# vitasoftAI/ImageRetrievalResearch

Hardware: AMD Instinct MI355X
Metric: images/sec embed + queries/sec top-k@100k-gallery, EffNet-B3a 224^2 (higher is better)
Workload: dtype bf16

## Files before the change

imageretrievalresearch_amd/csrc/common.h:

```cpp
#pragma once
#include <hip/hip_runtime.h>
#include <hip/hip_bf16.h>
#include <stdint.h>
#include <stdio.h>
#include <string>

namespace mi355 {

void set_error(const char* fmt, ...);
void roctx_enable(bool on);
bool roctx_active();
void roctx_push(const char* label);
void roctx_pop();
struct RoctxRange {
    bool on;
    explicit RoctxRange(const char* label) : on(label && roctx_active()) { if (on) roctx_push(label); }
    ~RoctxRange() { if (on) roctx_pop(); }
};
enum { OK = 0, ERR_ARG = 1, ERR_HIP = 2, ERR_STATE = 3, ERR_UNSUPPORTED = 4 };

#define MI355_CHECK_HIP(expr)                                                              \
    do {                                                                                   \
        hipError_t _e = (expr);                                                            \
        if (_e != hipSuccess) {                                                            \
            mi355::set_error("%s:%d: %s -> %s", __FILE__, __LINE__, #expr, hipGetErrorString(_e)); \
            return mi355::ERR_HIP;                                                         \
        }                                                                                  \
    } while (0)

#define MI355_REQUIRE(cond, ...)                                                           \
    do {                                                                                   \
        if (!(cond)) {                                                                     \
            mi355::set_error(__VA_ARGS__);                                                 \
            return mi355::ERR_ARG;                                                         \
        }                                                                                  \
    } while (0)

#define MI355_LAUNCH_CHECK() MI355_CHECK_HIP(hipGetLastError())

constexpr int MI355_MAX_DEVICES = 64;
static inline bool first_time_on_this_device(bool* flags) {
    int dev = 0;
    if (hipGetDevice(&dev) != hipSuccess || dev < 0 || dev >= MI355_MAX_DEVICES) return true;
    if (flags[dev]) return false;
    flags[dev] = true;
    return true;
}

static inline int cdiv(long a, long b) { return (int)((a + b - 1) / b); }
static inline size_t align_up(size_t a, size_t b) { return (a + b - 1) / b * b; }

static inline char* align256(const void* p) { return (char*)(((uintptr_t)p + 255) & ~(uintptr_t)255); }
struct WsCarver {
    char* base;
    size_t off = 0;
    explicit WsCarver(void* ws) : base(ws ? align256(ws) : nullptr) {}
    char* next() const { return base ? base + off : nullptr; }
    char* take(size_t bytes) { char* p = next(); off += align_up(bytes, 256); return p; }
    size_t total() const { return off + 256; }
};

typedef unsigned short bf16_t;

__device__ __forceinline__ float bf2f(bf16_t v) { return __uint_as_float(((unsigned)v) << 16); }
__device__ __forceinline__ bf16_t f2bf(float f) {
    __hip_bfloat16 h = __float2bfloat16(f);
    return *reinterpret_cast<bf16_t*>(&h);
}
typedef __bf16 mi355_bf16x2 __attribute__((ext_vector_type(2)));
typedef float mi355_f32x2 __attribute__((ext_vector_type(2)));
__device__ __forceinline__ unsigned pack2bf(float lo, float hi) {
    const mi355_bf16x2 v = __builtin_convertvector((mi355_f32x2){lo, hi}, mi355_bf16x2);
    return *reinterpret_cast<const unsigned*>(&v);
}

__device__ __forceinline__ float sigmoid_f(float x) {
    return __builtin_amdgcn_rcpf(1.0f + __builtin_amdgcn_exp2f(-1.4426950408889634f * x));
}
__device__ __forceinline__ float silu_f(float x) { return x * sigmoid_f(x); }

__device__ __forceinline__ float gelu_f(float x) {
    const float z = fabsf(x) * 0.70710678118654752f;
    const float t = __builtin_amdgcn_rcpf(1.0f + 0.3275911f * z);
    const float poly = ((((1.061405429f * t - 1.453152027f) * t + 1.421413741f) * t - 0.284496736f) * t + 0.254829592f) * t;
    const float e = 1.0f - poly * __builtin_amdgcn_exp2f(-1.4426950408889634f * z * z);
    return 0.5f * x * (1.0f + copysignf(e, x));
}

enum Act { ACT_NONE = 0, ACT_SILU = 1, ACT_RELU = 2, ACT_RELU6 = 3, ACT_GELU = 4, ACT_SIGMOID = 5 };

__device__ __forceinline__ float apply_act(float x, int act) {
    switch (act) {
        case ACT_SILU: return silu_f(x);
        case ACT_RELU: return fmaxf(x, 0.f);
        case ACT_RELU6: return fminf(fmaxf(x, 0.f), 6.f);
        case ACT_GELU: return gelu_f(x);
        case ACT_SIGMOID: return sigmoid_f(x);
        default: return x;
    }
}

template <int ACT>
__device__ __forceinline__ float act_c(float x) {
    if constexpr (ACT == ACT_SILU) return silu_f(x);
    else if constexpr (ACT == ACT_RELU) return fmaxf(x, 0.f);
    else if constexpr (ACT == ACT_RELU6) return fminf(fmaxf(x, 0.f), 6.f);
    else if constexpr (ACT == ACT_GELU) return gelu_f(x);
    else if constexpr (ACT == ACT_SIGMOID) return sigmoid_f(x);
    else return x;
}
#define MI355_ACT_DISPATCH(act_runtime, ...)                                      \
    switch (act_runtime) {                                                        \
        case ::mi355::ACT_SILU: { constexpr int ACT = ::mi355::ACT_SILU; __VA_ARGS__ } break;   \
        case ::mi355::ACT_GELU: { constexpr int ACT = ::mi355::ACT_GELU; __VA_ARGS__ } break;   \
        case ::mi355::ACT_RELU6: { constexpr int ACT = ::mi355::ACT_RELU6; __VA_ARGS__ } break; \
        case ::mi355::ACT_RELU: { constexpr int ACT = ::mi355::ACT_RELU; __VA_ARGS__ } break;   \
        case ::mi355::ACT_SIGMOID: { constexpr int ACT = ::mi355::ACT_SIGMOID; __VA_ARGS__ } break; \
        default: { constexpr int ACT = ::mi355::ACT_NONE; __VA_ARGS__ } break;    \
    }

__device__ __forceinline__ float wave_sum(float v) {
#pragma unroll
    for (int o = 32; o > 0; o >>= 1) v += __shfl_xor(v, o, 64);
    return v;
}
__device__ __forceinline__ float wave_max(float v) {
#pragma unroll
    for (int o = 32; o > 0; o >>= 1) v = fmaxf(v, __shfl_xor(v, o, 64));
    return v;
}

}
```

imageretrievalresearch_amd/csrc/conv_kernels.hip:

```cpp
#include "ops.h"
#include "../../include/mi355_retrieval.h"

#include <stdlib.h>
#include <type_traits>

namespace mi355 {

typedef float f32x4 __attribute__((ext_vector_type(4)));
typedef unsigned u32x4 __attribute__((ext_vector_type(4)));
typedef unsigned u32x2 __attribute__((ext_vector_type(2)));

__device__ __forceinline__ void unpack8(u32x4 v, float* f) {
    f[0] = __uint_as_float(v.x << 16); f[1] = __uint_as_float(v.x & 0xffff0000u);
    f[2] = __uint_as_float(v.y << 16); f[3] = __uint_as_float(v.y & 0xffff0000u);
    f[4] = __uint_as_float(v.z << 16); f[5] = __uint_as_float(v.z & 0xffff0000u);
    f[6] = __uint_as_float(v.w << 16); f[7] = __uint_as_float(v.w & 0xffff0000u);
}
__device__ __forceinline__ u32x4 pack8(const float* f) {
    u32x4 o;
    o.x = pack2bf(f[0], f[1]); o.y = pack2bf(f[2], f[3]); o.z = pack2bf(f[4], f[5]); o.w = pack2bf(f[6], f[7]);
    return o;
}

constexpr int STEM_TW = 16, STEM_TH = 16;
// ... 322 lines not shown
            }
        }
    }

    if (pool_partial != nullptr) {
#pragma unroll
        for (int j = 0; j < 8; ++j) red[threadIdx.x][j] = psum[j];
        __syncthreads();
        const int ncg = CG < 256 ? CG : 256;
        if ((int)threadIdx.x < ncg) {
            float s[8];
#pragma unroll
            for (int j = 0; j < 8; ++j) s[j] = 0.f;
            for (int u = threadIdx.x; u < 256; u += CG) {
#pragma unroll
                for (int j = 0; j < 8; ++j) s[j] += red[u][j];
            }
            const int my_cg = (int)(((long)blk * 256 + threadIdx.x) % CG);
            float* pp = pool_partial + ((size_t)b * nblk + blk) * C + my_cg * 8;
            *reinterpret_cast<f32x4*>(pp) = (f32x4){s[0], s[1], s[2], s[3]};
            *reinterpret_cast<f32x4*>(pp + 4) = (f32x4){s[4], s[5], s[6], s[7]};
        }
        if (CG > 256) {
            const int first = (int)(((long)blk * 256) % CG);
            for (int t = 256 + threadIdx.x; t < CG; t += 256) {
                const int z = (first + t) % CG;
                float* pp = pool_partial + ((size_t)b * nblk + blk) * C + z * 8;
                *reinterpret_cast<f32x4*>(pp) = (f32x4){0.f, 0.f, 0.f, 0.f};
                *reinterpret_cast<f32x4*>(pp + 4) = (f32x4){0.f, 0.f, 0.f, 0.f};
            }
        }
    }
}

template <int KS, int PX>
__global__ __launch_bounds__(256) void k_dw_tiled(const bf16_t* __restrict__ in, const bf16_t* __restrict__ w,
                                                  const float* __restrict__ bias, bf16_t* __restrict__ out,
                                                  float* __restrict__ pool_partial, int H, int W, int C, int TH, int CGC,
                                                  int nbands, int act) {
    constexpr int PAD = KS / 2;
    constexpr int IW = PX - 1 + KS;
    extern __shared__ __attribute__((aligned(16))) bf16_t tile[];
    const int b = blockIdx.y;
    const int band = blockIdx.x % nbands, chunk = blockIdx.x / nbands;
    const int oy0 = band * TH;
    const int th = min(TH, H - oy0);
    const int IH = TH + KS - 1, EW = W + 2 * PAD + (PX - 1);
    const int cg0 = chunk * CGC;
    const int CG = C >> 3;
    const int ncg = min(CGC, CG - cg0);
    const int PS = CGC * 8;
    const bf16_t* inb = in + (size_t)b * H * W * C;
    for (int id = threadIdx.x; id < IH * EW * CGC; id += 256) {
        const int cg = id % CGC;
        const int px = id / CGC;
        const int r = px / EW, x = px - r * EW;
        const int iy = oy0 - PAD + r, ix = x - PAD;
        u32x4 v = {0u, 0u, 0u, 0u};
        if (cg < ncg && iy >= 0 && iy < H && ix >= 0 && ix < W)
            v = *reinterpret_cast<const u32x4*>(inb + ((size_t)iy * W + ix) * C + (cg0 + cg) * 8);
        *reinterpret_cast<u32x4*>(&tile[(size_t)px * PS + cg * 8]) = v;
    }
    __syncthreads();

    const int strips = (W + PX - 1) / PX;
    const int nitems = CGC * strips * th;
    float psum[8];
#pragma unroll
    for (int j = 0; j < 8; ++j) psum[j] = 0.f;
    for (int item = threadIdx.x; item < nitems; item += 256) {
        const int cg = item % CGC;
        const int rest = item / CGC;
        const int sx = rest % strips, oyl = rest / strips;
        if (cg >= ncg) continue;
        const int ox0 = sx * PX;
        const int c0 = (cg0 + cg) * 8;
        float acc[PX][8];
        {
            const f32x4 b0 = *reinterpret_cast<const f32x4*>(bias + c0);
            const f32x4 b1 = *reinterpret_cast<const f32x4*>(bias + c0 + 4);
#pragma unroll
            for (int p = 0; p < PX; ++p) {
                acc[p][0] = b0.x; acc[p][1] = b0.y; acc[p][2] = b0.z; acc[p][3] = b0.w;
                acc[p][4] = b1.x; acc[p][5] = b1.y; acc[p][6] = b1.z; acc[p][7] = b1.w;
            }
        }
#pragma unroll
        for (int ky = 0; ky < KS; ++ky) {
            float wk[KS][8];
#pragma unroll
            for (int kx = 0; kx < KS; ++kx)
                unpack8(*reinterpret_cast<const u32x4*>(w + (size_t)(ky * KS + kx) * C + c0), wk[kx]);
            const bf16_t* row = tile + ((size_t)(oyl + ky) * EW + ox0) * PS + cg * 8;
#pragma unroll
            for (int i = 0; i < IW; ++i) {
                float v[8];
                unpack8(*reinterpret_cast<const u32x4*>(row + (size_t)i * PS), v);
#pragma unroll
                for (int p = 0; p < PX; ++p) {
                    const int kx = i - p;
                    if (kx >= 0 && kx < KS) {
#pragma unroll
                        for (int j = 0; j < 8; ++j) acc[p][j] += wk[kx][j] * v[j];
                    }
                }
            }
        }
        MI355_ACT_DISPATCH(act, {
_Pragma("unroll")
            for (int p = 0; p < PX; ++p)
_Pragma("unroll")
                for (int j = 0; j < 8; ++j) acc[p][j] = act_c<ACT>(acc[p][j]);
        })
        bf16_t* o = out + (((size_t)b * H + oy0 + oyl) * W + ox0) * C + c0;
#pragma unroll
        for (int p = 0; p < PX; ++p) {
            if (ox0 + p < W) {
#pragma unroll
                for (int j = 0; j < 8; ++j) psum[j] += acc[p][j];
                *reinterpret_cast<u32x4*>(o + (size_t)p * C) = pack8(acc[p]);
            }
        }
    }
    if (pool_partial != nullptr) {
        __syncthreads();
        float* red = reinterpret_cast<float*>(tile);
#pragma unroll
        for (int j = 0; j < 8; ++j) red[threadIdx.x * 8 + j] = psum[j];
        __syncthreads();
        if ((int)threadIdx.x < ncg) {
            float sacc[8] = {0.f, 0.f, 0.f, 0.f, 0.f, 0.f, 0.f, 0.f};
            for (int u = threadIdx.x; u < 256; u += CGC) {
#pragma unroll
                for (int j = 0; j < 8; ++j) sacc[j] += red[u * 8 + j];
            }
            float* pp = pool_partial + ((size_t)b * nbands + band) * C + (cg0 + threadIdx.x) * 8;
            *reinterpret_cast<f32x4*>(pp) = (f32x4){sacc[0], sacc[1], sacc[2], sacc[3]};
            *reinterpret_cast<f32x4*>(pp + 4) = (f32x4){sacc[4], sacc[5], sacc[6], sacc[7]};
        }
    }
}

static bool dw_tiled_plan(int H, int W, int C, int k, int stride, int* TH, int* CGC, int* PX, size_t* lds) {
    if (stride != 1 || W < 14 || C % 8) return false;
    const int CG = C / 8;
    const int cgc = CG < 8 ? CG : 8;
    const int px = W % 7 == 0 ? 7 : 4;
    const int strips = (W + px - 1) / px;
    int th = 256 / (cgc * strips);
    if (th < 1) return false;
    if (th > H) th = H;
    const int pad = k / 2;
    const size_t bytes = (size_t)(th + k - 1) * (W + 2 * pad + px - 1) * cgc * 16;
    if (bytes > 64 * 1024 || bytes < 256 * 8 * 4) return false;
    *TH = th; *CGC = cgc; *PX = px; *lds = bytes;
    return true;
}

template <int KS, int PX>
static int launch_dw_tiled(const bf16_t* in, const bf16_t* w, const float* bias, bf16_t* out, float* pool_partial, int B,
                           int H, int W, int C, int TH, int CGC, size_t lds, int act, int* pool_nblk, hipStream_t st) {
    static bool attr_done[MI355_MAX_DEVICES] = {false};
    if (first_time_on_this_device(attr_done)) {
        MI355_CHECK_HIP(hipFuncSetAttribute((const void*)k_dw_tiled<KS, PX>, hipFuncAttributeMaxDynamicSharedMemorySize,
                                            64 * 1024));
    }
    const int nbands = cdiv(H, TH), nchunks = cdiv(C / 8, CGC);
    hipLaunchKernelGGL((k_dw_tiled<KS, PX>), dim3(nbands * nchunks, B), dim3(256), lds, st, in, w, bias, out, pool_partial,
                       H, W, C, TH, CGC, nbands, act);
    MI355_LAUNCH_CHECK();
    if (pool_nblk) *pool_nblk = nbands;
    return OK;
}

typedef __bf16 dw_bf16x8 __attribute__((ext_vector_type(8)));
template <int NU>
__global__ __launch_bounds__(256, NU >= 6 ? 2 : (NU >= 4 ? 3 : 4)) void k_dw3_lds(
    const bf16_t* __restrict__ in, const bf16_t* __restrict__ w, const float* __restrict__ bias, bf16_t* __restrict__ out,
    float* __restrict__ pool_partial, int B, int nblk, int H, int W, int act, unsigned magicW, int tiles_per_wg) {
    constexpr int C = NU * 8, PB = C * 2;
    constexpr int ROWB = 34 * PB;
    constexpr int NCH = 3 * ROWB / 16;
    constexpr int NLD = (NCH + 63) / 64;
    constexpr int OUTB = 32 * PB, NOC = OUTB / 16, NST = (NOC + 63) / 64;
    constexpr int WS = 3 * ROWB + OUTB + NU * 16 + NU * 32;
    __shared__ __attribute__((aligned(16))) unsigned char lds[4 * WS];
    __shared__ float red[4][NU * 8];
    const int xcd = blockIdx.x & 7, seq = blockIdx.x >> 3;
    const int b = xcd + 8 * (seq / nblk), blk = seq - (seq / nblk) * nblk;
    if (b >= B) return;
    const int lane = threadIdx.x & 63;
    const int wave = __builtin_amdgcn_readfirstlane(threadIdx.x >> 6);
    const int fr = lane & 15, fq = lane >> 4;
    const int HW = H * W;
    unsigned char* Lw = lds + wave * WS;
    unsigned char* Lo = Lw + 3 * ROWB;
    unsigned char* Lz = Lo + OUTB;
    float* Lb = reinterpret_cast<float*>(Lz + NU * 16);
    if (lane < NU) *reinterpret_cast<u32x4*>(Lz + lane * 16) = (u32x4){0u, 0u, 0u, 0u};
    if (lane < NU * 8) Lb[lane] = bias[lane];
    u32x4 dwf[NU][3];
    {
        const int pm = fr >> 3, c = fr & 7, t = fq - pm;
        const int q = c >> 1;
#pragma unroll
        for (int u = 0; u < NU; ++u)
#pragma unroll
            for (int ky = 0; ky < 3; ++ky) {
                unsigned v = 0u;
                if (t >= 0 && t < 3) v = w[(size_t)(ky * 3 + t) * C + u * 8 + c];
                const unsigned word = (c & 1) ? (v << 16) : v;
                dwf[u][ky] = (u32x4){q == 0 ? word : 0u, q == 1 ? word : 0u, q == 2 ? word : 0u, q == 3 ? word : 0u};
            }
    }
    const int ch4 = (fq & 1) * 4, pp = fq >> 1;
    const bf16_t* img = in + (size_t)b * HW * C;
    const __amdgpu_buffer_rsrc_t rsrc = __builtin_amdgcn_make_buffer_rsrc(const_cast<bf16_t*>(img), 0, HW * PB, 0x00020000);
    unsigned char* ob = reinterpret_cast<unsigned char*>(out + (size_t)b * HW * C);
    const int rowb = W * PB;
    const int ntiles = (HW + 31) >> 5;
    const int t_end = min(ntiles, (blk + 1) * tiles_per_wg);
    float psum[NU][4];
#pragma unroll
    for (int u = 0; u < NU; ++u)
#pragma unroll
        for (int j = 0; j < 4; ++j) psum[u][j] = 0.f;
    int s_goff[NLD], s_loff[NLD];
#pragma unroll
    for (int i = 0; i < NLD; ++i) {
        const int ch = lane + 64 * i;
        const int ky = ch / (ROWB / 16), rem = ch - ky * (ROWB / 16);
        s_loff[i] = ch < NCH ? ky * ROWB + rem * 16 : -1;
        s_goff[i] = ch < NCH ? (ky - 1) * rowb + rem * 16 - PB : 0x40000000;
    }
    u32x4 sv[NLD];
    auto stage_load = [&](int tile) {
        const int base = tile * 32 * PB;
#pragma unroll
        for (int i = 0; i < NLD; ++i) sv[i] = __builtin_amdgcn_raw_buffer_load_b128(rsrc, base + s_goff[i], 0, 0);
        __builtin_amdgcn_sched_barrier(0);
    };
    const int t_begin = blk * tiles_per_wg + wave;
    if (t_begin < t_end) stage_load(t_begin);
    for (int tile = t_begin; tile < t_end; tile += 4) {
#pragma unroll
        for (int i = 0; i < NLD; ++i)
            if (s_loff[i] >= 0) *reinterpret_cast<u32x4*>(Lw + s_loff[i]) = sv[i];
        if (tile + 4 < t_end) stage_load(tile + 4);
        const int q = tile * 32 + 2 * fr;
        const int y = (int)__umulhi((unsigned)q, magicW);
        const int x = q - y * W;
        const bool colok = !(fq == 0 && x == 0) && !(fq == 3 && x == W - 2);
        const unsigned char* rb = Lw + (2 * fr + fq) * PB;
        const unsigned char* r0 = colok ? rb : Lz;
        const unsigned char* r1 = colok ? rb + ROWB : Lz;
        const unsigned char* r2 = colok ? rb + 2 * ROWB : Lz;
        const bool live = q + pp < HW;
#pragma unroll
        for (int u = 0; u < NU; ++u) {
            const u32x4 x0 = *reinterpret_cast<const u32x4*>(r0 + u * 16);
            const u32x4 x1 = *reinterpret_cast<const u32x4*>(r1 + u * 16);
            const u32x4 x2 = *reinterpret_cast<const u32x4*>(r2 + u * 16);
            f32x4 acc = *reinterpret_cast<const f32x4*>(Lb + u * 8 + ch4);
            acc = __builtin_amdgcn_mfma_f32_16x16x32_bf16(*reinterpret_cast<const dw_bf16x8*>(&dwf[u][0]), *reinterpret_cast<const dw_bf16x8*>(&x0), acc, 0, 0, 0);
            acc = __builtin_amdgcn_mfma_f32_16x16x32_bf16(*reinterpret_cast<const dw_bf16x8*>(&dwf[u][1]), *reinterpret_cast<const dw_bf16x8*>(&x1), acc, 0, 0, 0);
            acc = __builtin_amdgcn_mfma_f32_16x16x32_bf16(*reinterpret_cast<const dw_bf16x8*>(&dwf[u][2]), *reinterpret_cast<const dw_bf16x8*>(&x2), acc, 0, 0, 0);
            MI355_ACT_DISPATCH(act, {
                acc.x = act_c<ACT>(acc.x); acc.y = act_c<ACT>(acc.y); acc.z = act_c<ACT>(acc.z); acc.w = act_c<ACT>(acc.w);
            })
            if (live) { psum[u][0] += acc.x; psum[u][1] += acc.y; psum[u][2] += acc.z; psum[u][3] += acc.w; }
            u32x2 o;
            o.x = pack2bf(acc.x, acc.y);
            o.y = pack2bf(acc.z, acc.w);
            *reinterpret_cast<u32x2*>(Lo + (2 * fr + pp) * PB + u * 16 + ch4 * 2) = o;
        }
        const int nvalid = min(32, HW - tile * 32) * PB;
#pragma unroll
        for (int i = 0; i < NST; ++i) {
            const int ob_off = (lane + 64 * i) * 16;
            if (ob_off < nvalid && ob_off < OUTB)
                *reinterpret_cast<u32x4*>(ob + (size_t)tile * 32 * PB + ob_off) = *reinterpret_cast<const u32x4*>(Lo + ob_off);
        }
    }
    if (pool_partial) {
#pragma unroll
        for (int u = 0; u < NU; ++u) {
#pragma unroll
            for (int o = 1; o < 16; o <<= 1) {
#pragma unroll
                for (int j = 0; j < 4; ++j) psum[u][j] += __shfl_xor(psum[u][j], o, 64);
            }
#pragma unroll
            for (int j = 0; j < 4; ++j) psum[u][j] += __shfl_xor(psum[u][j], 32, 64);
            if (fr == 0 && fq < 2)
                *reinterpret_cast<f32x4*>(&red[wave][u * 8 + ch4]) = (f32x4){psum[u][0], psum[u][1], psum[u][2], psum[u][3]};
        }
        __syncthreads();
        if (threadIdx.x < NU * 8)
            pool_partial[((size_t)b * nblk + blk) * C + threadIdx.x] =
                ((red[0][threadIdx.x] + red[1][threadIdx.x]) + red[2][threadIdx.x]) + red[3][threadIdx.x];
    }
}

template <int NU>
static void launch_dw3_lds(const bf16_t* in, const bf16_t* w, const float* bias, bf16_t* out, float* pool_partial, int B, int nb,
                           int H, int W, int act, unsigned magic, int tpw, hipStream_t st) {
    hipLaunchKernelGGL((k_dw3_lds<NU>), dim3((unsigned)(8 * cdiv(B, 8) * nb)), dim3(256), 0, st, in, w, bias, out, pool_partial, B,
                       nb, H, W, act, magic, tpw);
}

bool dw_tiled_supported(int H, int W, int C, int k, int stride) {
    int TH, CGC, PX;
    size_t lds;
    return dw_tiled_plan(H, W, C, k, stride, &TH, &CGC, &PX, &lds);
}

bool dw3_lds_supported(int H, int W, int C, int k, int stride) {
    return k == 3 && stride == 1 && C <= 48 && W % 2 == 0 && W >= 4 && (long)H * W * C * 2 < (1L << 30);
}

void dw_env_choice(bool* try_tiled, bool* try_mfma) {
    static const int use_tiled = getenv("MI355_DW_TILED") ? atoi(getenv("MI355_DW_TILED")) : 0;
    static const int use_mfma = getenv("MI355_DW_MFMA") ? atoi(getenv("MI355_DW_MFMA")) : 1;
    *try_tiled = use_tiled != 0;
    *try_mfma = use_mfma != 0;
}

int launch_dwconv_sel(const bf16_t* in, const bf16_t* w, const float* bias, bf16_t* out, float* pool_partial, int B, int H,
                      int W, int C, int k, int stride, int act, bool try_tiled, bool try_mfma, int* pool_nblk, int* path,
                      hipStream_t st) {
    MI355_REQUIRE(C % 8 == 0, "dwconv: C=%d must be a multiple of 8", C);
    MI355_REQUIRE((k == 3 || k == 5) && (stride == 1 || stride == 2), "dwconv: unsupported k=%d stride=%d", k, stride);
    const int pad = k / 2;
    const int Ho = (H + 2 * pad - k) / stride + 1, Wo = (W + 2 * pad - k) / stride + 1;
    auto ran = [path](int p, int e) {
        if (path && e == OK) *path = p;
        return e;
    };
    int TH, CGC, PX;
    size_t lds;
    if (try_tiled && dw_tiled_plan(H, W, C, k, stride, &TH, &CGC, &PX, &lds)) {
        const int p = MI355_DW_PATH(MI355_DW_PATH_TILED, k, 1, PX, 0);
        if (k == 3) return ran(p, PX == 7 ? launch_dw_tiled<3, 7>(in, w, bias, out, pool_partial, B, H, W, C, TH, CGC, lds, act, pool_nblk, st)
                                          : launch_dw_tiled<3, 4>(in, w, bias, out, pool_partial, B, H, W, C, TH, CGC, lds, act, pool_nblk, st));
        return ran(p, PX == 7 ? launch_dw_tiled<5, 7>(in, w, bias, out, pool_partial, B, H, W, C, TH, CGC, lds, act, pool_nblk, st)
                              : launch_dw_tiled<5, 4>(in, w, bias, out, pool_partial, B, H, W, C, TH, CGC, lds, act, pool_nblk, st));
    }
    if (try_mfma && dw3_lds_supported(H, W, C, k, stride)) {
        const int ntiles = cdiv((long)H * W, 32);
        int nb = std::min(std::min(dw_pool_blocks(Ho, Wo, C), 14), ntiles);
        const int tpw = cdiv(ntiles, nb);
        nb = cdiv(ntiles, tpw);
        if (pool_nblk) *pool_nblk = nb;
        const unsigned magic = (unsigned)((0x100000000ULL + (unsigned)W - 1) / (unsigned)W);
        switch (C / 8) {
            case 1: launch_dw3_lds<1>(in, w, bias, out, pool_partial, B, nb, H, W, act, magic, tpw, st); break;
            case 2: launch_dw3_lds<2>(in, w, bias, out, pool_partial, B, nb, H, W, act, magic, tpw, st); break;
            case 3: launch_dw3_lds<3>(in, w, bias, out, pool_partial, B, nb, H, W, act, magic, tpw, st); break;
            case 4: launch_dw3_lds<4>(in, w, bias, out, pool_partial, B, nb, H, W, act, magic, tpw, st); break;
            case 5: launch_dw3_lds<5>(in, w, bias, out, pool_partial, B, nb, H, W, act, magic, tpw, st); break;
            default: launch_dw3_lds<6>(in, w, bias, out, pool_partial, B, nb, H, W, act, magic, tpw, st); break;
        }
        MI355_LAUNCH_CHECK();
        return ran(MI355_DW_PATH(MI355_DW_PATH_LDS3, 3, 1, C / 8, 0), OK);
    }
    if (pool_nblk) *pool_nblk = dw_pool_blocks(Ho, Wo, C);
    const int nblk = dw_pool_blocks(Ho, Wo, C);
    dim3 grid((unsigned)(8 * cdiv(B, 8) * nblk));
#define DW_LAUNCH(KS, S)                                                                                            \
    hipLaunchKernelGGL((k_dwconv<KS, S>), grid, dim3(256), 0, st, in, w, bias, out, pool_partial, B, nblk, H, W, C, Ho, Wo, act)
    if (k == 3 && stride == 1) DW_LAUNCH(3, 1);
    else if (k == 3 && stride == 2) DW_LAUNCH(3, 2);
    else if (k == 5 && stride == 1) DW_LAUNCH(5, 1);
    else DW_LAUNCH(5, 2);
#undef DW_LAUNCH
    MI355_LAUNCH_CHECK();
    return ran(MI355_DW_PATH(MI355_DW_PATH_DIRECT, k, stride, DW_PX, 0), OK);
}

int launch_dwconv(const bf16_t* in, const bf16_t* w, const float* bias, bf16_t* out, float* pool_partial, int B, int H,
                  int W, int C, int k, int stride, int act, int* pool_nblk, hipStream_t st) {
    bool try_tiled, try_mfma;
    dw_env_choice(&try_tiled, &try_mfma);
    return launch_dwconv_sel(in, w, bias, out, pool_partial, B, H, W, C, k, stride, act, try_tiled, try_mfma, pool_nblk, nullptr, st);
}

constexpr int SE_THREADS = 1024;
__global__ __launch_bounds__(SE_THREADS) void k_se(const float* __restrict__ pool_partial, int nblk, float inv_hw,
                                                   const float* __restrict__ w1, const float* __restrict__ b1,
                                                   const float* __restrict__ w2t, const float* __restrict__ b2,
                                                   float* __restrict__ gate, int C, int rd, int act1) {
    __shared__ float s[SE_MAX_C];
    __shared__ float r[SE_MAX_RD];
    const int b = blockIdx.x;
    const int tid = threadIdx.x, lane = tid & 63, wave = tid >> 6;
    const float* pp = pool_partial + (size_t)b * nblk * C;
    for (int c = tid; c < C; c += SE_THREADS) {
        float a = 0.f;
#pragma unroll 8
        for (int k = 0; k < nblk; ++k) a += pp[(size_t)k * C + c];
        s[c] = a * inv_hw;
    }
    __syncthreads();
    for (int jj = wave; jj < rd; jj += SE_THREADS / 64) {
        const int j = (jj + b) % rd;
        const float* wr = w1 + (size_t)j * C;
        float a = 0.f;
#pragma unroll 4
        for (int c = lane; c < C; c += 64) a += wr[c] * s[c];
        a = wave_sum(a);
        if (lane == 0) r[j] = apply_act(a + b1[j], act1);
    }
    __syncthreads();
    const int rot = (b * 192) % C;
    for (int cc = tid; cc < C; cc += SE_THREADS) {
        int c = cc + rot;
        if (c >= C) c -= C;
        float a = b2[c];
#pragma unroll 8
        for (int j = 0; j < rd; ++j) a += w2t[(size_t)j * C + c] * r[j];
        gate[(size_t)b * C + c] = sigmoid_f(a);
    }
}

__global__ __launch_bounds__(SE_THREADS) void k_se_small(const float* __restrict__ pool_partial, int nblk, float inv_hw,
                                                   const float* __restrict__ w1, const float* __restrict__ b1,
                                                   const float* __restrict__ w2t, const float* __restrict__ b2,
                                                   float* __restrict__ gate, int C, int rd, int act1) {
    __shared__ float s[SE_MAX_C];
    __shared__ float r[SE_MAX_RD];
    const int b = blockIdx.x;
    const int tid = threadIdx.x, lane = tid & 63, wave = tid >> 6;
    const float* pp = pool_partial + (size_t)b * nblk * C;
    for (int c = tid; c < C; c += SE_THREADS) {
        float a = 0.f;
#pragma unroll 8
        for (int k = 0; k < nblk; ++k) a += pp[(size_t)k * C + c];
        s[c] = a * inv_hw;
    }
    __syncthreads();
    constexpr int NBJ = 16;
    const int rot = (b * 192) % C;
    int c2 = (int)tid + rot;
    if (c2 >= C) c2 -= C;
    const bool has_c = (int)tid < C;
    float w2v[NBJ];
    float b2v = 0.f;
    if (has_c) {
        b2v = b2[c2];
#pragma unroll
        for (int t = 0; t < NBJ; ++t) w2v[t] = w2t[(size_t)min(t, rd - 1) * C + c2];
    }
    __builtin_amdgcn_sched_barrier(0);
    for (int jj = wave; jj < rd; jj += SE_THREADS / 64) {
        const int j = (jj + b) % rd;
        const float* wr = w1 + (size_t)j * C;
        const float bj = b1[j];
        float a = 0.f;
        constexpr int NBC = 8;
        for (int cb = 0; cb < C; cb += 64 * NBC) {
            float wv[NBC];
#pragma unroll
            for (int t = 0; t < NBC; ++t) wv[t] = wr[min(cb + t * 64 + lane, C - 1)];
#pragma unroll
            for (int t = 0; t < NBC; ++t) {
                const int c = cb + t * 64 + lane;
                a += c < C ? wv[t] * s[c] : 0.f;
            }
        }
        a = wave_sum(a);
        if (lane == 0) r[j] = apply_act(a + bj, act1);
    }
    __syncthreads();
    if (has_c) {
        float a = b2v;
#pragma unroll
        for (int t = 0; t < NBJ; ++t) a += t < rd ? w2v[t] * r[t] : 0.f;
        for (int j0 = NBJ; j0 < rd; j0 += NBJ) {
            float wv[NBJ];
#pragma unroll
            for (int t = 0; t < NBJ; ++t) wv[t] = w2t[(size_t)min(j0 + t, rd - 1) * C + c2];
#pragma unroll
            for (int t = 0; t < NBJ; ++t) a += j0 + t < rd ? wv[t] * r[j0 + t] : 0.f;
        }
        gate[(size_t)b * C + c2] = sigmoid_f(a);
    }
    for (int cc = tid + SE_THREADS; cc < C; cc += SE_THREADS) {
        int c = cc + rot;
        if (c >= C) c -= C;
        float a = b2[c];
        for (int j0 = 0; j0 < rd; j0 += NBJ) {
            float wv[NBJ];
#pragma unroll
            for (int t = 0; t < NBJ; ++t) wv[t] = w2t[(size_t)min(j0 + t, rd - 1) * C + c];
#pragma unroll
            for (int t = 0; t < NBJ; ++t) a += j0 + t < rd ? wv[t] * r[j0 + t] : 0.f;
        }
        gate[(size_t)b * C + c] = sigmoid_f(a);
    }
}

int launch_se(const float* pool_partial, int nblk, float inv_hw, const float* w1, const float* b1, const float* w2t,
              const float* b2, float* gate, int B, int C, int rd, int act1, hipStream_t st, int* path) {
    MI355_REQUIRE(C <= SE_MAX_C && rd <= SE_MAX_RD, "se: C=%d rd=%d exceed limits", C, rd);
    const bool small = rd <= 16 && C <= SE_THREADS;
    if (small)
        hipLaunchKernelGGL(k_se_small, dim3(B), dim3(SE_THREADS), 0, st, pool_partial, nblk, inv_hw, w1, b1, w2t, b2, gate, C, rd, act1);
    else
        hipLaunchKernelGGL(k_se, dim3(B), dim3(SE_THREADS), 0, st, pool_partial, nblk, inv_hw, w1, b1, w2t, b2, gate, C, rd, act1);
    MI355_LAUNCH_CHECK();
    if (path) *path = small ? MI355_DW_PATH_SE_SMALL : MI355_DW_PATH_SE_FULL;
    return OK;
}

__global__ __launch_bounds__(256) void k_gap(const bf16_t* __restrict__ in, float* __restrict__ pooled,
                                             bf16_t* __restrict__ pooled_bf16, int HW, int C, long total) {
    const long t = (long)blockIdx.x * 256 + threadIdx.x;
    if (t >= total) return;
    const int CG = C >> 3;
    const int cg = (int)(t % CG);
    const long b = t / CG;
    const bf16_t* p = in + (size_t)b * HW * C + cg * 8;
    float a[8] = {0, 0, 0, 0, 0, 0, 0, 0};
    for (int i = 0; i < HW; ++i) {
        float v[8];
        unpack8(*reinterpret_cast<const u32x4*>(p + (size_t)i * C), v);
#pragma unroll
        for (int j = 0; j < 8; ++j) a[j] += v[j];
    }
    const float inv = 1.0f / (float)HW;
#pragma unroll
    for (int j = 0; j < 8; ++j) a[j] *= inv;
    float* o = pooled + (size_t)b * C + cg * 8;
    *reinterpret_cast<f32x4*>(o) = (f32x4){a[0], a[1], a[2], a[3]};
    *reinterpret_cast<f32x4*>(o + 4) = (f32x4){a[4], a[5], a[6], a[7]};
    if (pooled_bf16) *reinterpret_cast<u32x4*>(pooled_bf16 + (size_t)b * C + cg * 8) = pack8(a);
}

int launch_gap(const bf16_t* in, float* pooled, bf16_t* pooled_bf16, int B, int HW, int C, hipStream_t st) {
    MI355_REQUIRE(C % 8 == 0, "gap: C=%d must be a multiple of 8", C);
    const long total = (long)B * (C / 8);
    hipLaunchKernelGGL(k_gap, dim3(cdiv(total, 256)), dim3(256), 0, st, in, pooled, pooled_bf16, HW, C, total);
    MI355_LAUNCH_CHECK();
    return OK;
}

__global__ __launch_bounds__(256) void k_pool_linear(const float* __restrict__ fm, const float* __restrict__ w,
                                                     const float* __restrict__ bias, float* __restrict__ out,
                                                     float* __restrict__ pooled_out, int C, int HW, int N) {
    extern __shared__ float pl[];
    const int b = blockIdx.x, tid = threadIdx.x, lane = tid & 63, wave = tid >> 6;
    const float* f = fm + (size_t)b * C * HW;
    const float inv = 1.0f / (float)HW;
    for (int c = tid; c < C; c += 256) {
        float a = 0.f;
        for (int i = 0; i < HW; ++i) a += f[(size_t)c * HW + i];
        a *= inv;
        if (pooled_out) pooled_out[(size_t)b * C + c] = a;
        pl[c] = bf2f(f2bf(a));
    }
    __syncthreads();
    if (w == nullptr) return;
    for (int n = wave; n < N; n += 4) {
        const float* wr = w + (size_t)n * C;
        float a = 0.f;
        for (int c = lane; c < C; c += 64) a += bf2f(f2bf(wr[c])) * pl[c];
        a = wave_sum(a);
        if (lane == 0) out[(size_t)b * N + n] = a + (bias ? bias[n] : 0.f);
    }
}

int launch_pool_linear(const float* fm, const float* w, const float* bias, float* out, float* pooled_out, int B, int C,
                       int HW, int N, hipStream_t st) {
    MI355_REQUIRE((size_t)C * 4 <= 64 * 1024, "pool_linear: C=%d too large", C);
    hipLaunchKernelGGL(k_pool_linear, dim3(B), dim3(256), (size_t)C * 4, st, fm, w, bias, out, pooled_out, C, HW, N);
    MI355_LAUNCH_CHECK();
    return OK;
}

__global__ __launch_bounds__(256) void k_nhwc_to_nchw(const bf16_t* __restrict__ in, float* __restrict__ out, int HW,
                                                      int C, int Cvalid) {
    __shared__ float tile[32][33];
    const int b = blockIdx.z;
    const int p0 = blockIdx.x * 32, c0 = blockIdx.y * 32;
    const int tx = threadIdx.x & 31, ty = threadIdx.x >> 5;
    for (int i = ty; i < 32; i += 8) {
        const int p = p0 + i, c = c0 + tx;
        tile[i][tx] = (p < HW && c < C) ? bf2f(in[((size_t)b * HW + p) * C + c]) : 0.f;
    }
    __syncthreads();
    for (int i = ty; i < 32; i += 8) {
        const int c = c0 + i, p = p0 + tx;
        if (c < Cvalid && p < HW) out[((size_t)b * Cvalid + c) * HW + p] = tile[tx][i];
    }
}

int launch_nhwc_to_nchw_f32(const bf16_t* in, float* out, int B, int HW, int C, int Cvalid, hipStream_t st) {
    dim3 grid(cdiv(HW, 32), cdiv(C, 32), B);
    hipLaunchKernelGGL(k_nhwc_to_nchw, grid, dim3(256), 0, st, in, out, HW, C, Cvalid);
    MI355_LAUNCH_CHECK();
    return OK;
}

__global__ __launch_bounds__(256) void k_nchw_to_nhwc(const float* __restrict__ in, bf16_t* __restrict__ out, int HW,
                                                      int Cvalid, int C) {
    __shared__ float tile[32][33];
    const int b = blockIdx.z;
    const int p0 = blockIdx.x * 32, c0 = blockIdx.y * 32;
    const int tx = threadIdx.x & 31, ty = threadIdx.x >> 5;
    for (int i = ty; i < 32; i += 8) {
        const int c = c0 + i, p = p0 + tx;
// ... 82 lines not shown
```

imageretrievalresearch_amd/csrc/sweep_mbconv.hip:

```cpp
#include "../../include/mi355_retrieval.h"
#include "ops.h"
#include <type_traits>

namespace mi355 {

typedef __bf16 bf16x8 __attribute__((ext_vector_type(8)));
typedef float f32x4 __attribute__((ext_vector_type(4)));
typedef unsigned u32x4 __attribute__((ext_vector_type(4)));
typedef unsigned u32x2 __attribute__((ext_vector_type(2)));

__device__ __forceinline__ void sw_lds_barrier() {
    asm volatile("s_waitcnt lgkmcnt(0)" ::: "memory");
    __builtin_amdgcn_s_barrier();
    asm volatile("" ::: "memory");
}

__device__ __forceinline__ void sw_dma16(const void* gsrc, unsigned lds_dst) {
    unsigned keep;
    asm volatile("s_mov_b32 %0, m0\n\ts_mov_b32 m0, %2\n\ts_nop 0\n\tglobal_load_lds_dwordx4 %1, off\n\ts_mov_b32 m0, %0"
                 : "=&s"(keep) : "v"(gsrc), "s"(lds_dst) : "memory");
}
__device__ __forceinline__ void sw_dma4(const void* gsrc, unsigned lds_dst) {
    unsigned keep;
    asm volatile("s_mov_b32 %0, m0\n\ts_mov_b32 m0, %2\n\ts_nop 0\n\tglobal_load_lds_dword %1, off\n\ts_mov_b32 m0, %0"
                 : "=&s"(keep) : "v"(gsrc), "s"(lds_dst) : "memory");
}

template <int N>
__device__ __forceinline__ void sw_wait_vm_leaving(int n) {
    if constexpr (N == 0) asm volatile("s_waitcnt vmcnt(0)" ::: "memory");
    else {
        if (n >= N) asm volatile("s_waitcnt vmcnt(%0)" ::"n"(N) : "memory");
        else sw_wait_vm_leaving<N - 1>(n);
    }
}

typedef __bf16 sw_bf16x2 __attribute__((ext_vector_type(2)));
typedef float sw_f32x2 __attribute__((ext_vector_type(2)));
__device__ __forceinline__ u32x2 sw_pack4(const f32x4 v) {
    const sw_bf16x2 lo = __builtin_convertvector((sw_f32x2){v.x, v.y}, sw_bf16x2);
    const sw_bf16x2 hi = __builtin_convertvector((sw_f32x2){v.z, v.w}, sw_bf16x2);
    u32x2 o;
    o.x = *reinterpret_cast<const unsigned*>(&lo);
    o.y = *reinterpret_cast<const unsigned*>(&hi);
    return o;
}

template <int ACT>
__device__ __forceinline__ float sw_act(float x, int act_runtime) {
    if constexpr (ACT >= 0) return act_c<ACT>(x);
    else return apply_act(x, act_runtime);
}

template <int KS> struct SwTaps {
    static constexpr int NV = (KS / 2) * KS;
    static constexpr int NH = (KS + 1) / 2;
    static constexpr int NP = NV + NH;
    __host__ __device__ static constexpr bool vertical(int tp) { return tp < NV; }
    __host__ __device__ static constexpr int tap_a(int tp) {
        return tp < NV ? (tp / KS) * 2 * KS + tp % KS : (KS - 1) * KS + (tp - NV) * 2;
    }
    __host__ __device__ static constexpr int tap_b(int tp) {
        return tp < NV ? tap_a(tp) + KS : ((tp - NV) * 2 + 1 < KS ? tap_a(tp) + 1 : -1);
    }
};

template <int KS, int S, int WI, int TH>
struct SwGeom {
    static constexpr int PAD = KS / 2;
    static constexpr int HALO = KS - S;
    static constexpr int NEWR = TH * S;
    static constexpr int IH = NEWR + HALO;
    static constexpr int EW = WI + 2 * PAD;
    static constexpr int EWH = (EW + 1) / 2;
    static constexpr int RP = S == 1 ? EW : 2 * EWH;
    static constexpr int HOFF = S == 1 ? 1 : EWH;
    static constexpr int WO = (WI + 2 * PAD - KS) / S + 1;
    static constexpr int ELD = 24;
    static constexpr int EBUF = (IH + 1) * RP * ELD;
    static constexpr int NWD = (KS * KS * 8 + 63) / 64;
    static constexpr int cst_bytes(int kst) { return kst * 1024 + 128 + NWD * 256; }
    static constexpr size_t lds_bytes(int nw, int ns, int kst, int nwalk) {
        return (size_t)2 * ns * cst_bytes(kst) + (size_t)ns * 2 * EBUF * 2 + (size_t)nwalk * nw * 16 * ns * 4;
    }
    __host__ __device__ static constexpr int epx(int r, int c) {
        return r * RP + (S == 1 ? c : (c & 1) * EWH + (c >> 1));
    }
};

template <int KS, int S, int WI, int TH, int NW, int KST, int OCC, bool PREF, int AE, int AD, int NS = 1>
__global__ __launch_bounds__(NW * 64, (NW * OCC + 3) / 4) void k_sweep_mbconv(const SweepArgs a) {
    using G = SwGeom<KS, S, WI, TH>;
    using TP = SwTaps<KS>;
    constexpr int NTHR = NW * 64;
    constexpr int PAD = G::PAD, HALO = G::HALO, NEWR = G::NEWR, RP = G::RP, ELD = G::ELD, WO = G::WO, NP = TP::NP;
    constexpr int NPX1 = NEWR * WI, NT1 = (NPX1 + 15) / 16, MW1 = (NT1 + NW - 1) / NW;
    constexpr int NPX2 = TH * WO, NT2 = (NPX2 + 15) / 16, MW2 = (NT2 + NW - 1) / NW;
    constexpr int EBUF = G::EBUF;
    extern __shared__ __attribute__((aligned(16))) unsigned char sw_smem[];
    constexpr int NWD = G::NWD, CST = G::cst_bytes(KST);
    const unsigned char* cst = sw_smem;
    bf16_t* Es = reinterpret_cast<bf16_t*>(sw_smem + 2 * NS * CST);
    float* red = reinterpret_cast<float*>(sw_smem + 2 * NS * CST + (size_t)NS * 2 * EBUF * 2);

    const int tid = threadIdx.x, lane = tid & 63;
    const int wave = __builtin_amdgcn_readfirstlane(tid >> 6);
    const int fr = lane & 15, fq = lane >> 4;
    const int xcd = blockIdx.x & 7, seq = blockIdx.x >> 3;
    const int b = xcd + 8 * (seq / a.csplit), g = seq % a.csplit;
    if (b >= a.B) return;
    const int midp = (a.mid + 15) & ~15;
    const int nslab = (midp / 16 + NS - 1) / NS;
    const int nbands = (a.Ho + TH - 1) / TH;

    const bool stamping = a.stamps != nullptr;
    long long t_acc[10] = {0, 0, 0, 0, 0, 0, 0, 0, 0, 0};
    long long t_last = 0;
    if (stamping) t_last = (long long)__builtin_readcyclecounter();
    auto tick = [&](int i) {
        if (stamping) { const long long t = (long long)__builtin_readcyclecounter(); t_acc[i] += t - t_last; t_last = t; }
    };

    const bf16_t* xb = a.X + (size_t)b * a.H * WI * a.Cin;
    bf16_t* Db = a.D + (size_t)b * a.Ho * WO * a.mid;
    const int hw1 = a.H * WI - 1;
    const int kclamp = a.Cin - 8;

    u32x4 xa[MW1][KST];
    auto load_x_of = [&](int band, auto first) {
        constexpr bool FIRST = decltype(first)::value;
        const int pix0 = (band * NEWR - PAD + HALO) * WI;
        int l = lane;
        if constexpr (FIRST) asm volatile("" : "+v"(l));
        const int lr = l & 15, lk = (l >> 4) * 8;
#pragma unroll
        for (int i = 0; i < MW1; ++i) {
            const int pix = min(max(pix0 + (wave + NW * i) * 16 + lr, 0), hw1);
#pragma unroll
            for (int ks = 0; ks < KST; ++ks) {
                u32x4 t = {0u, 0u, 0u, 0u};
                if (!(a.debug_skip & 4)) t = *reinterpret_cast<const u32x4*>(xb + pix * a.Cin + min(ks * 32 + lk, kclamp));
                xa[i][ks] = t;
            }
        }
        __builtin_amdgcn_sched_barrier(0);
    };

    auto ch0_of = [&](int si) { return ((si + b) % nslab) * (16 * NS); };
    const unsigned cst_lds = (unsigned)(size_t)(__attribute__((address_space(3))) unsigned char*)sw_smem;
    auto stage_consts = [&](int ch0, int set) {
        int l = lane;
        asm volatile("" : "+v"(l));
        const int lr = l & 15, lk = (l >> 4) * 8;
#pragma unroll
        for (int s = 0; s < NS; ++s) {
            const int c0 = ch0 + 16 * s;
            const unsigned dst = cst_lds + (set * NS + s) * CST;
            const int n = min(c0 + lr, midp - 1);
#pragma unroll
            for (int ks = 0; ks < KST; ++ks) sw_dma16(a.We + (n * a.Kp + ks * 32 + lk), dst + ks * 1024);
            if (l < 8) {
                const int q = l & 3;
                const float* src = l < 4 ? a.be + min(c0 + q * 4, midp - 4) : a.bd + min(c0 + q * 4, a.mid - 4);
                sw_dma16(src, dst + KST * 1024);
            }
#pragma unroll
            for (int j = 0; j < NWD; ++j) {
                const int t = min(j * 8 + (l >> 3), KS * KS - 1);
                sw_dma4(a.Wd + (t * a.mid + min(c0 + 2 * (l & 7), a.mid - 2)), dst + KST * 1024 + 128 + j * 256);
            }
        }
    };
    u32x4 wf[NS][KST];
    f32x4 bb[NS];
    if (wave == NW - 1) stage_consts(ch0_of(g), 0);
    if (PREF) load_x_of(-1, std::true_type{});

    for (int id = tid; id < NS * 2 * EBUF / 8; id += NTHR) *reinterpret_cast<u32x4*>(&Es[id * 8]) = (u32x4){0u, 0u, 0u, 0u};

    int eoff[MW1];
#pragma unroll
    for (int i = 0; i < MW1; ++i) {
        const int p = min((wave + NW * i) * 16 + fr, NPX1 - 1);
        const int r = p / WI, x = p - r * WI;
        eoff[i] = G::epx(HALO + r, x + PAD) * ELD + fq * 4;
    }
    int rbase[MW2];
#pragma unroll
    for (int i = 0; i < MW2; ++i) {
        const int p = min((wave + NW * i) * 16 + fr, NPX2 - 1);
        const int oyl = p / WO, ox = p - oyl * WO;
        rbase[i] = (oyl * S * RP + ox) * ELD + (fq & 1) * 8;
    }
    const int vsel = (fq >> 1) ? RP * ELD : 0;
    const int hsel = (fq >> 1) ? G::HOFF * ELD : 0;
    if (wave == NW - 1) asm volatile("s_waitcnt vmcnt(0)" ::: "memory");
    sw_lds_barrier();
    tick(0);

    int pb = 0;
    int kslab = 0;
    int nst = 0;
    for (int si = g; si < nslab; si += a.csplit, ++kslab) {
        const int ch0 = ch0_of(si);
        const bool has_next = si + a.csplit < nslab;
        if constexpr (HALO > NEWR) {
            constexpr int NZ16 = (HALO - NEWR) * RP * ELD / 8;
#pragma unroll
            for (int s = 0; s < NS; ++s)
                for (int id = tid; id < NZ16; id += NTHR)
                    *reinterpret_cast<u32x4*>(&Es[(s * 2 + pb) * EBUF + NEWR * RP * ELD + id * 8]) = (u32x4){0u, 0u, 0u, 0u};
        }
        if (!PREF) load_x_of(-1, std::true_type{});
        f32x4 bdr[NS];
        unsigned wd_raw[NS][(NP + 1) / 2];
        int l = lane;
        asm volatile("" : "+v"(l));
#pragma unroll
        for (int s = 0; s < NS; ++s) {
            const unsigned char* cs = cst + ((kslab & 1) * NS + s) * CST;
#pragma unroll
            for (int ks = 0; ks < KST; ++ks) wf[s][ks] = *reinterpret_cast<const u32x4*>(cs + ks * 1024 + l * 16);
            bb[s] = *reinterpret_cast<const f32x4*>(cs + KST * 1024 + (l >> 4) * 16);
            bdr[s] = *reinterpret_cast<const f32x4*>(cs + KST * 1024 + 64 + (l >> 4) * 16);
            const unsigned short* wds = reinterpret_cast<const unsigned short*>(cs + KST * 1024 + 128) + (l & 15);
#pragma unroll
            for (int tp = 0; tp < NP; ++tp) {
                const int ta = TP::tap_a(tp), tb = TP::tap_b(tp) < 0 ? TP::tap_a(tp) : TP::tap_b(tp);
                const unsigned v = wds[((l & 32) ? tb : ta) * 16];
                if (tp & 1) wd_raw[s][tp >> 1] |= v << 16;
                else wd_raw[s][tp >> 1] = v;
            }
        }
        if (PREF) sw_wait_vm_leaving<MW2 * NS>(nst);
        else asm volatile("s_waitcnt vmcnt(0)" ::: "memory");
#pragma unroll
        for (int i = 0; i < MW1; ++i)
#pragma unroll
            for (int ks = 0; ks < KST; ++ks) asm volatile("" : "+v"(xa[i][ks]));
        if (has_next && wave == NW - 1) stage_consts(ch0_of(si + a.csplit), (kslab + 1) & 1);
        auto build_dwf = [&](int s, u32x4* dwf) {
            const bool mine = ((fq & 1) == (fr >> 3)) && (ch0 + 16 * s + fr < a.mid);
            const int q = (fr & 7) >> 1;
#pragma unroll
            for (int tp = 0; tp < NP; ++tp) {
                const bool has = mine && !((lane & 32) && TP::tap_b(tp) < 0);
                const unsigned v = has ? ((tp & 1) ? wd_raw[s][tp >> 1] >> 16 : wd_raw[s][tp >> 1] & 0xffffu) : 0u;
                const unsigned word = (fr & 1) ? (v << 16) : v;
                dwf[tp] = (u32x4){q == 0 ? word : 0u, q == 1 ? word : 0u, q == 2 ? word : 0u, q == 3 ? word : 0u};
            }
        };
        constexpr bool DWF_PER_SLAB = KS == 3;
        u32x4 dwf_s[NS][DWF_PER_SLAB ? NP : 1];
        float psum[NS][4];
#pragma unroll
        for (int s = 0; s < NS; ++s)
#pragma unroll
            for (int j = 0; j < 4; ++j) psum[s][j] = 0.f;
        if constexpr (DWF_PER_SLAB) {
#pragma unroll
            for (int s = 0; s < NS; ++s) build_dwf(s, dwf_s[s]);
        }
        tick(1);

        for (int band = -1; band < nbands; ++band) {
            bf16_t* Ec = Es + ((band + 1 + pb) & 1) * EBUF;
            {
                const int iyn0 = band * NEWR - PAD + HALO;
                const int plo = max(0, -iyn0) * WI, phi = max(0, min(NEWR, a.H - iyn0)) * WI;
                if (!PREF && band >= 0) load_x_of(band, std::false_type{});
                tick(3);
                if (stamping) { asm volatile("s_waitcnt vmcnt(0)" ::: "memory"); tick(4); }
#pragma unroll
                for (int i = 0; i < MW1; ++i) {
                    const int t0 = (wave + NW * i) * 16;
                    if (t0 < NPX1 && (band >= 0 || t0 + 16 > (NEWR - HALO) * WI)) {
#pragma unroll
                        for (int s = 0; s < NS; ++s) {
                            u32x2 o = {0u, 0u};
                            if (t0 < phi && t0 + 16 > plo && !(a.debug_skip & 1)) {
                                f32x4 acc = bb[s];
#pragma unroll
                                for (int ks = 0; ks < KST; ++ks)
                                    acc = __builtin_amdgcn_mfma_f32_16x16x32_bf16(*reinterpret_cast<bf16x8*>(&wf[s][ks]),
                                                                                  *reinterpret_cast<bf16x8*>(&xa[i][ks]), acc, 0, 0, 0);
                                acc.x = sw_act<AE>(acc.x, a.act_e); acc.y = sw_act<AE>(acc.y, a.act_e);
                                acc.z = sw_act<AE>(acc.z, a.act_e); acc.w = sw_act<AE>(acc.w, a.act_e);
                                o = sw_pack4(acc);
                                if (t0 < plo || t0 + 16 > phi) {
                                    const bool in = t0 + fr >= plo && t0 + fr < phi;
                                    o.x = in ? o.x : 0u; o.y = in ? o.y : 0u;
                                }
                            }
                            if (t0 + fr < NPX1) *reinterpret_cast<u32x2*>(&Ec[s * 2 * EBUF + eoff[i]]) = o;
                        }
                    }
                }
                const bool last = band + 1 >= nbands;
                if (last && has_next && wave == NW - 1) asm volatile("s_waitcnt vmcnt(0)" ::: "memory");
                if (PREF && (!last || has_next)) {
                    load_x_of(last ? -1 : band + 1, std::false_type{});
                    if (last) nst = 0;
                }
            }
            tick(5);
            sw_lds_barrier();
            tick(6);
            if (band + 1 < nbands) {
                bf16_t* En = Es + ((band + pb) & 1) * EBUF;
                constexpr int NV16 = HALO * RP * ELD / 8;
#pragma unroll
                for (int s = 0; s < NS; ++s)
                    for (int id = tid; id < NV16; id += NTHR)
                        *reinterpret_cast<u32x4*>(&En[s * 2 * EBUF + id * 8]) = *reinterpret_cast<const u32x4*>(&Ec[s * 2 * EBUF + NEWR * RP * ELD + id * 8]);
            }
            tick(2);
#pragma unroll
            for (int s = 0; s < NS; ++s) {
            const int c0 = ch0 + 16 * s;
            if (band >= 0 && c0 < a.mid && !(a.debug_skip & 2)) {
                u32x4 dwf_b[DWF_PER_SLAB ? 1 : NP];
                if constexpr (!DWF_PER_SLAB) build_dwf(s, dwf_b);
                const u32x4* dwf = DWF_PER_SLAB ? dwf_s[s] : dwf_b;
                const int np2 = min(TH, a.Ho - band * TH) * WO;
// ... 212 lines not shown
```

Before: 62450.

## Stream depthwise 3x3 input through an LDS ring buffer with async DMA

Adds a depthwise 3x3 stride-1 kernel that keeps a power-of-two ring of input pixels in LDS. The ring is filled with global_load_lds DMA in 1KB chunks and refilled ahead of compute, so each workgroup streams its rows instead of staging a full tile per step. Output goes through a per-wave LDS buffer and buffer stores, and pooling partial sums are fused in. The old LDS kernel stays as the fallback when the ring cannot hold two rows plus margin. Shared DMA helpers move to common.h for reuse.

```diff
diff --git a/imageretrievalresearch_amd/csrc/common.h b/imageretrievalresearch_amd/csrc/common.h
--- a/imageretrievalresearch_amd/csrc/common.h
+++ b/imageretrievalresearch_amd/csrc/common.h
@@ -130,4 +130,16 @@
     return v;
 }
 
+__device__ __forceinline__ void sw_lds_barrier() {
+    asm volatile("s_waitcnt lgkmcnt(0)" ::: "memory");
+    __builtin_amdgcn_s_barrier();
+    asm volatile("" ::: "memory");
 }
+
+__device__ __forceinline__ void sw_dma16(const void* gsrc, unsigned lds_dst) {
+    unsigned keep;
+    asm volatile("s_mov_b32 %0, m0\n\ts_mov_b32 m0, %2\n\ts_nop 0\n\tglobal_load_lds_dwordx4 %1, off\n\ts_mov_b32 m0, %0"
+                 : "=&s"(keep) : "v"(gsrc), "s"(lds_dst) : "memory");
+}
+
+}
diff --git a/imageretrievalresearch_amd/csrc/conv_kernels.hip b/imageretrievalresearch_amd/csrc/conv_kernels.hip
--- a/imageretrievalresearch_amd/csrc/conv_kernels.hip
+++ b/imageretrievalresearch_amd/csrc/conv_kernels.hip
@@ -648,11 +648,147 @@
     }
 }
 
+constexpr int DW3_RING_PX = 512;
+static bool dw3_ring_fits(int W, int C) {
+    return (2 * W + 258) * (C * 2) + 1023 <= DW3_RING_PX * (C * 2);
+}
+
+template <int NU>
+__global__ __launch_bounds__(256, NU >= 6 ? 2 : (NU >= 4 ? 3 : 4)) void k_dw3_ring(
+    const bf16_t* __restrict__ in, const bf16_t* __restrict__ w, const float* __restrict__ bias, bf16_t* __restrict__ out,
+    float* __restrict__ pool_partial, int B, int nblk, int H, int W, int act, unsigned magicW, int tiles_per_wg) {
+    constexpr int C = NU * 8, PB = C * 2;
+    constexpr int RP = DW3_RING_PX, RB = RP * PB, NCHK = RB / 1024;
+    static_assert((RP & (RP - 1)) == 0 && RB % 1024 == 0, "ring: a power of two of pixels, whole pieces");
+    constexpr int OUTB = 32 * PB, NOC = OUTB / 16, NST = (NOC + 63) / 64;
+    __shared__ __attribute__((aligned(1024))) unsigned char lds[RB + NU * 16 + NU * 32 + 4 * OUTB];
+    __shared__ float red[4][NU * 8];
+    const int xcd = blockIdx.x & 7, seq = blockIdx.x >> 3;
+    const int b = xcd + 8 * (seq / nblk), blk = seq - (seq / nblk) * nblk;
+    if (b >= B) return;
+    const int lane = threadIdx.x & 63;
+    const int wave = __builtin_amdgcn_readfirstlane(threadIdx.x >> 6);
+    const int fr = lane & 15, fq = lane >> 4;
+    const int HW = H * W;
+    unsigned char* Lr = lds;
+    unsigned char* Lz = lds + RB;
+    float* Lb = reinterpret_cast<float*>(Lz + NU * 16);
+    unsigned char* Lo = Lz + NU * 16 + NU * 32 + wave * OUTB;
+    if (threadIdx.x < NU) *reinterpret_cast<u32x4*>(Lz + threadIdx.x * 16) = (u32x4){0u, 0u, 0u, 0u};
+    if (threadIdx.x < NU * 8) Lb[threadIdx.x] = bias[threadIdx.x];
+    u32x4 dwf[NU][3];
+    {
+        const int pm = fr >> 3, c = fr & 7, t = fq - pm;
+        const int q = c >> 1;
+#pragma unroll
+        for (int u = 0; u < NU; ++u)
+#pragma unroll
+            for (int ky = 0; ky < 3; ++ky) {
+                unsigned v = 0u;
+                if (t >= 0 && t < 3) v = w[(size_t)(ky * 3 + t) * C + u * 8 + c];
+                const unsigned word = (c & 1) ? (v << 16) : v;
+                dwf[u][ky] = (u32x4){q == 0 ? word : 0u, q == 1 ? word : 0u, q == 2 ? word : 0u, q == 3 ? word : 0u};
+            }
+    }
+    const int ch4 = (fq & 1) * 4, pp = fq >> 1;
+    const unsigned char* imgb = reinterpret_cast<const unsigned char*>(in + (size_t)b * HW * C);
+    const int img_bytes = HW * PB;
+    const __amdgpu_buffer_rsrc_t orsrc = __builtin_amdgcn_make_buffer_rsrc(out + (size_t)b * HW * C, 0, img_bytes, 0x00020000);
+    const int ntiles = (HW + 31) >> 5;
+    const int T0 = blk * tiles_per_wg;
+    const int t_end = min(ntiles, T0 + tiles_per_wg);
+    const int nsteps = (t_end - T0 + 3) >> 2;
+    float psum[NU][4];
+#pragma unroll
+    for (int u = 0; u < NU; ++u)
+#pragma unroll
+        for (int j = 0; j < 4; ++j) psum[u][j] = 0.f;
+    const int lo0 = (T0 * 32 - W - 1) * PB;
+    const int c_end = ((t_end * 32 + W + 1) * PB + 1023) >> 10;
+    const unsigned ring_lds = (unsigned)(size_t)(__attribute__((address_space(3))) unsigned char*)lds;
+    int c_next = lo0 >> 10;
+    auto request_to = [&](int c_hi) {
+        for (int c = c_next + ((wave - c_next) & 3); c < c_hi; c += 4) {
+            const unsigned slot = (unsigned)((c + 64 * NCHK) % NCHK) * 1024u;
+            const int g = c * 1024 + lane * 16;
+            if (g >= 0 && g < img_bytes) sw_dma16(imgb + g, ring_lds + slot);
+            else *reinterpret_cast<u32x4*>(Lr + slot + lane * 16) = (u32x4){0u, 0u, 0u, 0u};
+        }
+        c_next = max(c_next, c_hi);
+    };
+    request_to(min(c_end, c_next + NCHK));
+    for (int s = 0; s < nsteps; ++s) {
+        if (s == 0) asm volatile("s_waitcnt vmcnt(0)" ::: "memory");
+        else asm volatile("s_waitcnt vmcnt(%0)" ::"n"(NST) : "memory");
+        sw_lds_barrier();
+        if (s > 0) request_to(min(c_end, ((lo0 + s * 128 * PB) >> 10) + NCHK));
+        const int tile = T0 + 4 * s + wave;
+        if (tile < t_end) {
+            const int q = tile * 32 + 2 * fr;
+            const int y = (int)__umulhi((unsigned)q, magicW);
+            const int x = q - y * W;
+            const bool colok = !(fq == 0 && x == 0) && !(fq == 3 && x == W - 2);
+            const int p1 = q + fq - 1;
+            const unsigned char* r0 = colok ? Lr + ((p1 - W) & (RP - 1)) * PB : Lz;
+            const unsigned char* r1 = colok ? Lr + (p1 & (RP - 1)) * PB : Lz;
+            const unsigned char* r2 = colok ? Lr + ((p1 + W) & (RP - 1)) * PB : Lz;
+            const bool live = q + pp < HW;
+#pragma unroll
+            for (int u = 0; u < NU; ++u) {
+                const u32x4 x0 = *reinterpret_cast<const u32x4*>(r0 + u * 16);
+                const u32x4 x1 = *reinterpret_cast<const u32x4*>(r1 + u * 16);
+                const u32x4 x2 = *reinterpret_cast<const u32x4*>(r2 + u * 16);
+                f32x4 acc = *reinterpret_cast<const f32x4*>(Lb + u * 8 + ch4);
+                acc = __builtin_amdgcn_mfma_f32_16x16x32_bf16(*reinterpret_cast<const dw_bf16x8*>(&dwf[u][0]), *reinterpret_cast<const dw_bf16x8*>(&x0), acc, 0, 0, 0);
+                acc = __builtin_amdgcn_mfma_f32_16x16x32_bf16(*reinterpret_cast<const dw_bf16x8*>(&dwf[u][1]), *reinterpret_cast<const dw_bf16x8*>(&x1), acc, 0, 0, 0);
+                acc = __builtin_amdgcn_mfma_f32_16x16x32_bf16(*reinterpret_cast<const dw_bf16x8*>(&dwf[u][2]), *reinterpret_cast<const dw_bf16x8*>(&x2), acc, 0, 0, 0);
+                MI355_ACT_DISPATCH(act, {
+                    acc.x = act_c<ACT>(acc.x); acc.y = act_c<ACT>(acc.y); acc.z = act_c<ACT>(acc.z); acc.w = act_c<ACT>(acc.w);
+                })
+                if (live) { psum[u][0] += acc.x; psum[u][1] += acc.y; psum[u][2] += acc.z; psum[u][3] += acc.w; }
+                u32x2 o;
+                o.x = pack2bf(acc.x, acc.y);
+                o.y = pack2bf(acc.z, acc.w);
+                *reinterpret_cast<u32x2*>(Lo + (2 * fr + pp) * PB + u * 16 + ch4 * 2) = o;
+            }
+#pragma unroll
+            for (int i = 0; i < NST; ++i) {
+                const int ob_off = (lane + 64 * i) * 16;
+                const bool ok = ob_off < OUTB;
+                const u32x4 v = *reinterpret_cast<const u32x4*>(Lo + (ok ? ob_off : 0));
+                __builtin_amdgcn_raw_buffer_store_b128(v, orsrc, ok ? tile * 32 * PB + ob_off : 0x40000000, 0, 0);
+            }
+        }
+    }
+    asm volatile("s_waitcnt vmcnt(0)" ::: "memory");
+    if (pool_partial) {
+#pragma unroll
+        for (int u = 0; u < NU; ++u) {
+#pragma unroll
+            for (int o = 1; o < 16; o <<= 1) {
+#pragma unroll
+                for (int j = 0; j < 4; ++j) psum[u][j] += __shfl_xor(psum[u][j], o, 64);
+            }
+#pragma unroll
+            for (int j = 0; j < 4; ++j) psum[u][j] += __shfl_xor(psum[u][j], 32, 64);
+            if (fr == 0 && fq < 2)
+                *reinterpret_cast<f32x4*>(&red[wave][u * 8 + ch4]) = (f32x4){psum[u][0], psum[u][1], psum[u][2], psum[u][3]};
+        }
+        __syncthreads();
+        if (threadIdx.x < NU * 8)
+            pool_partial[((size_t)b * nblk + blk) * C + threadIdx.x] =
+                ((red[0][threadIdx.x] + red[1][threadIdx.x]) + red[2][threadIdx.x]) + red[3][threadIdx.x];
+    }
+}
+
 template <int NU>
 static void launch_dw3_lds(const bf16_t* in, const bf16_t* w, const float* bias, bf16_t* out, float* pool_partial, int B, int nb,
                            int H, int W, int act, unsigned magic, int tpw, hipStream_t st) {
-    hipLaunchKernelGGL((k_dw3_lds<NU>), dim3((unsigned)(8 * cdiv(B, 8) * nb)), dim3(256), 0, st, in, w, bias, out, pool_partial, B,
-                       nb, H, W, act, magic, tpw);
+    const dim3 grid((unsigned)(8 * cdiv(B, 8) * nb));
+    if (dw3_ring_fits(W, NU * 8))
+        hipLaunchKernelGGL((k_dw3_ring<NU>), grid, dim3(256), 0, st, in, w, bias, out, pool_partial, B, nb, H, W, act, magic, tpw);
+    else
+        hipLaunchKernelGGL((k_dw3_lds<NU>), grid, dim3(256), 0, st, in, w, bias, out, pool_partial, B, nb, H, W, act, magic, tpw);
 }
 
 bool dw_tiled_supported(int H, int W, int C, int k, int stride) {
diff --git a/imageretrievalresearch_amd/csrc/sweep_mbconv.hip b/imageretrievalresearch_amd/csrc/sweep_mbconv.hip
--- a/imageretrievalresearch_amd/csrc/sweep_mbconv.hip
+++ b/imageretrievalresearch_amd/csrc/sweep_mbconv.hip
@@ -9,17 +9,6 @@
 typedef unsigned u32x4 __attribute__((ext_vector_type(4)));
 typedef unsigned u32x2 __attribute__((ext_vector_type(2)));
 
-__device__ __forceinline__ void sw_lds_barrier() {
-    asm volatile("s_waitcnt lgkmcnt(0)" ::: "memory");
-    __builtin_amdgcn_s_barrier();
-    asm volatile("" ::: "memory");
-}
-
-__device__ __forceinline__ void sw_dma16(const void* gsrc, unsigned lds_dst) {
-    unsigned keep;
-    asm volatile("s_mov_b32 %0, m0\n\ts_mov_b32 m0, %2\n\ts_nop 0\n\tglobal_load_lds_dwordx4 %1, off\n\ts_mov_b32 m0, %0"
-                 : "=&s"(keep) : "v"(gsrc), "s"(lds_dst) : "memory");
-}
 __device__ __forceinline__ void sw_dma4(const void* gsrc, unsigned lds_dst) {
     unsigned keep;
     asm volatile("s_mov_b32 %0, m0\n\ts_mov_b32 m0, %2\n\ts_nop 0\n\tglobal_load_lds_dword %1, off\n\ts_mov_b32 m0, %0"
```

Measured after the change: 62900 (median of 6 runs). About the same (+0.7%).
